# zju3dv/disprcnn

Measured on AMD Instinct MI355X. Metric: ROI cost-volumes/sec (112x112x48), higher is better.
Workload: dtype f32 (every convolution of the regressor, the three 32->1 heads included: split-f16 -- each fp32 value carried as hi + lo fp16, 3 f16-MFMA products per fp32 product, f32 accumulate; fp32-class error, tests/test_hip_s16.py.  Head gather and soft-argmin: f32 VALU); 1 GPU; Config A: per ROI pair, features [32,28,28]x2 -> concat cost volume [64,12,28,28] (folded into the first 3D layer's loads, never written) -> 3D stacked-hourglass regressor -> trilinear x4 + softmax + soft-argmin -> disparity [112,112]; maxdisp=48, mindisp=0, parallelism=roi-shard x1 (no collective), weights=closed-form synthetic (disprcnn_amd.utils.synth), BN stats calibrated fixture

## Files before the change

disprcnn_amd/csrc/convs16.hip:

```cpp
#include <hip/hip_runtime.h>
#include <stdint.h>

#include <type_traits>

#include "../../include/disprcnn_hip.h"
#include "s16_cvrows.h"
#include "s16_ovf.h"
#include "s16_tilemap.h"

typedef float f32x4 __attribute__((ext_vector_type(4)));
typedef float f32x16 __attribute__((ext_vector_type(16)));
typedef unsigned u32x4 __attribute__((ext_vector_type(4)));
typedef unsigned u32x2 __attribute__((ext_vector_type(2)));
typedef _Float16 f16x8 __attribute__((ext_vector_type(8)));
typedef _Float16 f16x4 __attribute__((ext_vector_type(4)));

#define GLOBAL_PTR(p) ((const __attribute__((address_space(1))) void*)(p))
#define LDS_PTR(p) ((__attribute__((address_space(3))) void*)(p))
#define S16_WAITCNT(vm, lgkm) (((vm) & 15) | (7 << 4) | ((lgkm) << 8) | (((vm) >> 4) << 14))

namespace {

constexpr int PV_ROWS = 128;
constexpr int PV_FLAT = 192;
constexpr int RING = 3;

template <int KW, bool CV, int RT_ = 1, int WT = 28, bool RES = false, bool Y32 = false, bool HEAD = false>
__global__ __launch_bounds__(256) __attribute__((amdgpu_waves_per_eu(1, 1))) void convs16_kernel(const drc_s16conv_params p) {
    constexpr bool FL = RT_ == 0;
    constexpr int RT = FL ? 1 : RT_;
    static_assert(!HEAD || (KW == 2 && !CV && RT == 1 && !RES && !Y32), "the fused cout-1 head is a form of the 32 -> 32 full-resolution layer");
    static_assert(!CV || (KW == 4 && RT == 1 && WT == 28 && !RES && !Y32), "the cost-volume form: 64 virtual input channels, full-resolution rows, RS16 output");
    extern __shared__ __attribute__((aligned(16))) char lds[];
    if constexpr (CV) {
        s16cv::s16_cvrows_run<1>(p, lds);
        return;
    }
    constexpr int TX = WT;
    constexpr int SX = WT + 2;
    constexpr int RPW = 4 / KW;
    constexpr int CBI = KW / 2;
    constexpr int SROWS = RPW * RT + 2;
    static_assert(RT * WT <= 32, "tile shape");
    static_assert(!FL || (KW == 2 && !CV && WT == 28 && !Y32 && !HEAD), "flat tiles: the plain / residual 32 -> 32 layer on 28-column maps");
    constexpr int PV = FL ? PV_FLAT : PV_ROWS;
    constexpr int CPB = PV * 16;
    constexpr int NH = PV / 64;
    constexpr int SLAB = CBI * 8 * CPB;
    constexpr int NL = CBI * 8 * NH / 4;
    constexpr int OWN = 16 / KW;
    constexpr int XW = 4096;
    constexpr int NR = RES ? 2 : 0;
    constexpr int NS = 2;
    static_assert(!(Y32 && (KW != 2 || RES)), "the blocked fp32 output exists for the 32-channel layers without residual");
    static_assert(FL || (RT == 1 ? SROWS * SX + 4 <= PV : (SROWS + 1) * SX + 4 <= PV), "slab plane too small (incl. the rows / columns the idle lanes over-read)");
    char* ring = lds;
    char* xchg = lds + RING * SLAB;
    char* pbuf = xchg + 2 * 4 * XW;

    const int wave = __builtin_amdgcn_readfirstlane(threadIdx.x >> 6);
    const int lane = threadIdx.x & 63;
    const int n_ = lane & 31, g = lane >> 5;
    const S16TileLane tln = s16_tile_lane<RT, WT>(n_, !(p.lo4 & 0x100));
    const int rl = tln.rl, xl = tln.xl;
    const int r = wave / KW, k = wave % KW;
    const int n_ct = p.cout / 32;
    const int ct = (int)((blockIdx.x >> 3) % n_ct);

    const int D = p.D, H = p.H, W = p.W;
    const int Wp = W + 2, Hp = H + 2;
    const long rowB = (long)Wp * 128;
    const long planeB = (long)Hp * rowB;
    const long xcbB = (long)(D + 2) * planeB;
    const long xnB = (long)CBI * xcbB;
    const int cbo = p.cout / 32;
    const long ynB = (long)cbo * xcbB;
    const long b_rowB = (long)Wp * 64, b_planeB = (long)Hp * b_rowB, b_cbB = (long)(D + 2) * b_planeB, b_nB = (long)(p.cout / 16) * b_cbB;

    f16x8 wh[27], wl[27];
    {
        const char* wb = (const char*)p.w + ((long)(ct * KW + k) * 54) * 1024 + lane * 16;
#pragma unroll
        for (int t = 0; t < 27; ++t) {
            wh[t] = *(const f16x8*)(wb + (t * 2) * 1024);
            wl[t] = *(const f16x8*)(wb + (t * 2 + 1) * 1024);
        }
    }
    constexpr int PIN_WH = 14;
#pragma unroll
    for (int t = 0; t < 27; ++t) {
        asm volatile("" : "+a"(wl[t]));
        if (t < PIN_WH) asm volatile("" : "+a"(wh[t]));
    }
    float sc[OWN], sh[OWN];
#pragma unroll
    for (int e = 0; e < OWN; ++e) {
        const int reg = k * OWN + e;
        const int co = ct * 32 + (reg & 3) + 8 * (reg >> 2) + 4 * g;
        sc[e] = p.scale[co];
        sh[e] = p.shift[co];
    }
    f16x8 w1h = {}, w1l = {};
    if constexpr (HEAD) {
        const char* wb = (const char*)p.w1 + (long)k * 2048 + lane * 16;
        w1h = *(const f16x8*)wb;
        w1l = *(const f16x8*)(wb + 1024);
    }
    int srcrow[2], srcx[2];
    bool srcok[2];
#pragma unroll
    for (int h = 0; h < 2; ++h) {
        const int v = h * 64 + lane;
        srcok[h] = v < SROWS * SX;
        const int rr = srcok[h] ? v / SX : 0;
        srcrow[h] = rr;
        srcx[h] = srcok[h] ? v - rr * SX : 0;
    }
    const unsigned bfrag0 = (unsigned)(((k >> 1) * 8 + (k & 1) * 2 + g) * CPB);
    const unsigned bfrag = bfrag0 + (unsigned)(((r * RT + rl) * SX + xl) * 16);
    const __attribute__((address_space(3))) char* ringl = (const __attribute__((address_space(3))) char*)ring;
    typedef const __attribute__((address_space(3))) f16x8 lds_frag;

    const int n_xt = (W + TX - 1) / TX, n_yt = (H + RPW * RT - 1) / (RPW * RT);
    const int Dw = (D + 2) / 3 * 3;
    const unsigned xcd = blockIdx.x & 7, qx = (blockIdx.x >> 3) / n_ct, per_xcd = (gridDim.x >> 3) / n_ct;
    const int HW = H * W, Hp1 = H + 1;
    const unsigned G = FL ? ((p.dil & 0x4000) ? 1u : 4u) : 1u;
    const unsigned cols_unit = FL ? (G * (unsigned)HW + 63u) / 64u : (unsigned)n_yt * n_xt;

    struct Col { unsigned n; int y0, x0; bool valid; int rem0, lim; };
    auto col_of = [&](unsigned it) __attribute__((always_inline)) {
        const unsigned j = it * per_xcd + qx;
        const unsigned nl = j / cols_unit;
        const unsigned rem = j - nl * cols_unit;
        if constexpr (FL) {
            Col c;
            const unsigned n0 = (nl * 8 + xcd) * G;
            const int gu = n0 < (unsigned)p.N ? (int)((unsigned)p.N - n0 < G ? (unsigned)p.N - n0 : G) : 0;
            const int f0 = (int)rem * 64;
            const int u0 = f0 / HW;
            c.valid = f0 < gu * HW;
            c.n = n0 + (unsigned)u0;
            c.rem0 = f0 - u0 * HW;
            c.lim = gu * HW - f0;
            c.y0 = c.rem0 / WT;
            c.x0 = c.rem0 - c.y0 * WT;
            return c;
        }
        const int yb = (int)(rem / n_xt), xt = (int)(rem - (unsigned)yb * n_xt);
        Col c;
        c.n = nl * 8 + xcd;
        c.valid = c.n < (unsigned)p.N;
        c.y0 = yb * RPW * RT;
        c.x0 = xt * TX;
        c.rem0 = c.lim = 0;
        return c;
    };
    struct Src { const char* a; unsigned v0, v1, v2, v3; };
    auto src_of = [&](const Col& c) __attribute__((always_inline)) {
        Src q;
        q.a = (const char*)p.x + (long)c.n * xnB;
        q.v2 = q.v3 = 0u;
        if constexpr (FL) {
            const int el = c.rem0 + (c.lim < 64 ? c.lim : 64) - 1;
            const int du_l = (el >= HW) + (el >= 2 * HW) + (el >= 3 * HW);
            const int rr_last = du_l * Hp1 + (el - du_l * HW) / WT - c.y0 + 2;
            static_assert(NH <= 4, "pieces of a chunk plane");
            unsigned vv[4] = {0u, 0u, 0u, 0u};
#pragma unroll
            for (int h = 0; h < NH; ++h) {
                const int v = h * 64 + lane;
                const int rr = v / SX, xs = v - rr * SX;
                const int L = c.y0 + rr, M = L - 1;
                const int uo = (M >= Hp1) + (M >= 2 * Hp1) + (M >= 3 * Hp1);
                const unsigned off = (unsigned)((long)uo * xnB + (long)(L - uo * Hp1) * rowB + (long)xs * 16);
                vv[h] = rr <= rr_last ? off : 0x80000000u;
            }
            q.v0 = vv[0]; q.v1 = vv[1]; q.v2 = vv[2]; q.v3 = vv[3];
            return q;
        }
        q.v0 = (unsigned)((long)(c.y0 + srcrow[0]) * rowB + (long)(c.x0 + srcx[0]) * 16);
        q.v1 = (unsigned)((long)(c.y0 + srcrow[1]) * rowB + (long)(c.x0 + srcx[1]) * 16);
        return q;
    };
    auto stage = [&](const Src& q, int pl, int slot) __attribute__((always_inline)) {
        char* dst = ring + slot * SLAB;
        const __amdgpu_buffer_rsrc_t ra = __builtin_amdgcn_make_buffer_rsrc((void*)q.a, 0, 0x7FFFFF00, 0x00020000);
        const unsigned va[4] = {q.v0, q.v1, q.v2, q.v3};
#pragma unroll
        for (int i = 0; i < NL; ++i) {
            const int id = wave * NL + i;
            const int cb = FL ? 0 : id >> 4, c = FL ? wave * (NL / NH) + i / NH : (id >> 1) & 7, h = FL ? i % NH : id & 1;
            const int so = (int)((long)cb * xcbB + (long)(pl + 1) * planeB + (long)c * (Wp * 16));
            __builtin_amdgcn_raw_ptr_buffer_load_lds(ra, LDS_PTR(dst + (cb * 8 + c) * CPB + h * 1024), 16, va[h], so, 0, 0);
        }
    };
    const bool hrows = HEAD && p.head_rows;
    const int hs_slotB = hrows ? 16 : 48;
    const long hs_planeB = (long)H * W * hs_slotB, hs_nB = (long)D * hs_planeB;
    const bool hs_drop0 = hrows && g, hs_drop1 = hrows || g;
    struct Ctx { char* y16b; char* y32b; const char* resb; char* hsb; unsigned o16, o32, ohs, bf; bool ok; };
    auto ctx_of = [&](const Col& c) __attribute__((always_inline)) {
        Ctx q;
        q.bf = bfrag;
        if constexpr (FL) {
            q.hsb = (char*)p.w;
            q.y32b = (char*)p.w;
            q.ohs = q.o32 = 0u;
            q.y16b = (char*)p.y16 + (long)c.n * ynB;
            q.resb = p.res ? (const char*)p.res + (long)c.n * ynB : (const char*)p.w;
            q.ok = r * 32 + n_ < c.lim;
            const int e0 = q.ok ? c.rem0 + r * 32 + n_ : c.rem0;
            const int du = (e0 >= HW) + (e0 >= 2 * HW) + (e0 >= 3 * HW);
            const int e = e0 - du * HW;
            const int yl = e / WT, xv = e - yl * WT;
            q.bf = bfrag0 + (unsigned)(((du * Hp1 + yl - c.y0) * SX + xv) * 16);
            q.o16 = (unsigned)((long)du * ynB + (long)ct * xcbB + planeB + (long)(yl + 1) * rowB + (long)(k * 2 + g) * (Wp * 16) + (long)(xv + 1) * 16);
            return q;
        }
        q.hsb = HEAD ? (char*)p.head + (long)c.n * hs_nB : (char*)p.w;
        q.ohs = (unsigned)(((long)(c.y0 + r * RT + rl) * W + (c.x0 + xl)) * hs_slotB + (hrows ? 0 : g * 32));
        q.y16b = p.y16 ? (char*)p.y16 + (long)c.n * ynB : (char*)p.w;
        q.y32b = p.y32 ? (char*)p.y32 + (long)c.n * b_nB : (char*)p.w;
        q.resb = p.res ? (const char*)p.res + (long)c.n * ynB : (const char*)p.w;
        const int yl = c.y0 + r * RT + rl;
        q.ok = tln.ok && yl < H && c.x0 + xl < W;
        if constexpr (KW == 2) {
            q.o16 = (unsigned)((long)ct * xcbB + planeB + (long)(yl + 1) * rowB + (long)(k * 2 + g) * (Wp * 16) + (long)(c.x0 + xl + 1) * 16);
            q.o32 = (unsigned)((long)(2 * ct + k) * b_cbB + b_planeB + (long)(yl + 1) * b_rowB + (long)(c.x0 + xl + 1) * 64 + g * 16);
        } else {
            q.o16 = (unsigned)((long)ct * xcbB + planeB + (long)(yl + 1) * rowB + (long)((k >> 1) * 2 + g) * (Wp * 16) + (long)(c.x0 + xl + 1) * 16 + (k & 1) * 8);
            q.o32 = (unsigned)((long)(2 * ct + (k >> 1)) * b_cbB + b_planeB + (long)(yl + 1) * b_rowB + (long)(c.x0 + xl + 1) * 64 + (k & 1) * 32 + g * 16);
        }
        return q;
    };
    const unsigned lo_off = (unsigned)(4 * Wp * 16);
    const float relu_lo = p.relu ? 0.f : -65504.f;
    const unsigned n16 = p.y16 ? 0x7FFFFF00u : 0u, n32 = p.y32 ? 0x7FFFFF00u : 0u, nres = p.res ? 0x7FFFFF00u : 0u;

    Col ccur = col_of(0);
    if (!ccur.valid) return;
    S16Ovf og;
#pragma unroll
    for (int e = 0; e < OWN; ++e) { og.see_raw(sc[e], 3.0e38f); og.see_raw(sh[e], 3.0e38f); }
    Src s_cur = src_of(ccur), s_next = s_cur;
    Ctx cx_cur = ctx_of(ccur), cx_prev = cx_cur;
    cx_prev.ok = false;

    f32x16 acc[3];
    u32x4 resv[3][2];
#pragma unroll
    for (int a_ = 0; a_ < 3; ++a_)
#pragma unroll
        for (int e = 0; e < 16; ++e) acc[a_][e] = 0.f;
#pragma unroll
    for (int a_ = 0; a_ < 3; ++a_) resv[a_][0] = resv[a_][1] = (u32x4){0u, 0u, 0u, 0u};
    f32x16 pkeep = {};
    float SC[5] = {0.f, 0.f, 0.f, 0.f, 0.f}, SB[5] = {0.f, 0.f, 0.f, 0.f, 0.f};
    auto head_pack = [&](const float* o) __attribute__((always_inline)) {
        const bool live = n_ < WT;
        int v_[5];
#pragma unroll
        for (int j = 0; j < 5; ++j) v_[j] = __builtin_bit_cast(int, live ? o[j] : 0.f);
        auto left = [](int a) __attribute__((always_inline)) { return __builtin_bit_cast(float, __builtin_amdgcn_update_dpp(0, a, 0x138, 0xf, 0xf, true)); };
        auto right = [](int a) __attribute__((always_inline)) { return __builtin_bit_cast(float, __builtin_amdgcn_update_dpp(0, a, 0x130, 0xf, 0xf, true)); };
        auto own = [](int a) __attribute__((always_inline)) { return __builtin_bit_cast(float, a); };
        const float a0 = (left(v_[0]) + own(v_[1])) + right(v_[2]);
        const float a1 = left(v_[3]) + own(v_[4]);
        const float b0 = right(v_[0]);
        const float b1 = (left(v_[1]) + own(v_[2])) + right(v_[3]);
        const unsigned x0 = __builtin_amdgcn_permlane32_swap(__builtin_bit_cast(unsigned, b0), 0u, false, false)[1];
        const unsigned x1 = __builtin_amdgcn_permlane32_swap(__builtin_bit_cast(unsigned, b1), 0u, false, false)[1];
        u32x4 d;
        d[0] = hrows ? __builtin_bit_cast(unsigned, a0) : __builtin_bit_cast(unsigned, o[0]);
        d[1] = hrows ? __builtin_bit_cast(unsigned, a1) : __builtin_bit_cast(unsigned, o[1]);
        d[2] = hrows ? x0 : __builtin_bit_cast(unsigned, o[2]);
        d[3] = hrows ? x1 : __builtin_bit_cast(unsigned, o[3]);
        return d;
    };
    stage(s_cur, 0, 0);
    stage(s_cur, 1 < D ? 1 : D, 1);
    __builtin_amdgcn_s_waitcnt(S16_WAITCNT(NL, 15));
    unsigned gs = 0;

    auto step = [&](int t, auto JT, auto KT) __attribute__((always_inline)) {
        constexpr int J = decltype(JT)::value;
        constexpr int KIND = decltype(KT)::value;
        constexpr bool COMPUTE = KIND != 3;
        constexpr int A0 = (J + 1) % 3, A1 = J, A2 = (J + 2) % 3;
        asm volatile("" ::: "memory");
        __builtin_amdgcn_s_waitcnt(S16_WAITCNT(NL + NS + NR, 0));
        __builtin_amdgcn_s_barrier();
        asm volatile("" ::: "memory");
        const bool fcur = t >= 2, pcur = t >= 1;
        const int qf = fcur ? t - 2 : Dw - 2 + t, qp = pcur ? t - 1 : Dw - 1;
        const __amdgpu_buffer_rsrc_t resr = __builtin_amdgcn_make_buffer_rsrc((void*)(pcur ? cx_cur.resb : cx_prev.resb), 0, nres, 0x00020000);
        const unsigned p_o16 = pcur ? cx_cur.o16 : cx_prev.o16;
        const bool p_ok = (pcur ? cx_cur.ok : cx_prev.ok) && qp >= 0 && qp < D;
        if constexpr (RES) {
            const unsigned po = p_ok ? (unsigned)((long)qp * planeB) : 0x80000000u;
            if constexpr (KW == 2) {
                resv[J][0] = __builtin_amdgcn_raw_buffer_load_b128(resr, p_o16 + po, 0, 0);
                resv[J][1] = __builtin_amdgcn_raw_buffer_load_b128(resr, p_o16 + lo_off + po, 0, 0);
            } else {
                const u32x2 a_ = __builtin_amdgcn_raw_buffer_load_b64(resr, p_o16 + po, 0, 0);
                const u32x2 b_ = __builtin_amdgcn_raw_buffer_load_b64(resr, p_o16 + lo_off + po, 0, 0);
                resv[J][0] = (u32x4){a_.x, a_.y, 0u, 0u};
                resv[J][1] = (u32x4){b_.x, b_.y, 0u, 0u};
            }
        }
        {
            const int tp = t + 2;
            const bool nxt = tp >= Dw;
            Src q;
            q.a = nxt ? s_next.a : s_cur.a;
            q.v0 = nxt ? s_next.v0 : s_cur.v0;
            q.v1 = nxt ? s_next.v1 : s_cur.v1;
            q.v2 = nxt ? s_next.v2 : s_cur.v2;
            q.v3 = nxt ? s_next.v3 : s_cur.v3;
            int pl = nxt ? tp - Dw : tp;
            pl = pl < D ? pl : D;
            stage(q, pl, (J + 2) % 3);
        }
        const __amdgpu_buffer_rsrc_t y16r = __builtin_amdgcn_make_buffer_rsrc(fcur ? cx_cur.y16b : cx_prev.y16b, 0, n16, 0x00020000);
        const __amdgpu_buffer_rsrc_t y32r = __builtin_amdgcn_make_buffer_rsrc(fcur ? cx_cur.y32b : cx_prev.y32b, 0, n32, 0x00020000);
        const unsigned f_o16 = fcur ? cx_cur.o16 : cx_prev.o16, f_o32 = fcur ? cx_cur.o32 : cx_prev.o32;
        const bool f_ok = (fcur ? cx_cur.ok : cx_prev.ok) && qf >= 0 && qf < D;
        f32x4 part[4];
        {
            const char* xb = xchg + ((gs - 1) & 1) * (4 * XW) + (r * KW) * XW + lane * 16;
            if constexpr (KW == 2) {
                part[0] = *(const f32x4*)(xb + (k * 2) * 1024);
                part[1] = *(const f32x4*)(xb + XW + (k * 2) * 1024);
                part[2] = *(const f32x4*)(xb + (k * 2 + 1) * 1024);
                part[3] = *(const f32x4*)(xb + XW + (k * 2 + 1) * 1024);
            } else {
#pragma unroll
                for (int q = 0; q < 4; ++q) part[q] = *(const f32x4*)(xb + q * XW + k * 1024);
            }
        }
        f32x4 pin[4];
        if constexpr (HEAD) {
            const char* pb = pbuf + ((gs - 1) & 1) * (2 * XW) + r * XW + lane * 16;
#pragma unroll
            for (int q = 0; q < 4; ++q) pin[q] = *(const f32x4*)(pb + q * 1024);
        }
        if constexpr (RES) {
            __builtin_amdgcn_s_waitcnt(S16_WAITCNT(2 * NL + NS + NR, 15));
            __builtin_amdgcn_sched_barrier(0);
        }
        float v[OWN];
        _Float16 vh[OWN], vl[OWN];
        const unsigned long long og_keep = S16Ovf::lanes(f_ok);
        auto fin = [&](int e) __attribute__((always_inline)) {
            float s_;
            if constexpr (KW == 2) s_ = part[(e >> 2) * 2][e & 3] + part[(e >> 2) * 2 + 1][e & 3];
            else s_ = (part[0][e] + part[1][e]) + (part[2][e] + part[3][e]);
            float x_ = s_ * sc[e] + sh[e];
            if constexpr (RES) {
                const _Float16 rh = __builtin_bit_cast(f16x8, resv[(J + 2) % 3][0])[e], rl_ = __builtin_bit_cast(f16x8, resv[(J + 2) % 3][1])[e];
                x_ += (float)rh + (float)rl_;
            }
            x_ = __builtin_amdgcn_fmed3f(x_, relu_lo, 65504.f);
            og.see(x_, og_keep);
            v[e] = x_;
            vh[e] = (_Float16)x_;
            vl[e] = (_Float16)(x_ - (float)vh[e]);
        };
        auto stores = [&]() __attribute__((always_inline)) {
            if constexpr (Y32) {
// ... 25 lines not shown
#pragma unroll
            for (int e = 0; e < 16; ++e) acc[A2][e] = 0.f;
        };
        float o_[5];
        f32x16 z_ = {};
        f16x8 bh_ = {}, bl_ = {};
        auto head_update = [&](int jj) __attribute__((always_inline)) {
            if constexpr (HEAD) {
                const bool first = t == 3;
                const float p0 = pkeep[3 * jj] + pin[(3 * jj) >> 2][(3 * jj) & 3];
                const float p1 = pkeep[3 * jj + 1] + pin[(3 * jj + 1) >> 2][(3 * jj + 1) & 3];
                const float p2 = pkeep[3 * jj + 2] + pin[(3 * jj + 2) >> 2][(3 * jj + 2) & 3];
                o_[jj] = SC[jj] + (first ? 0.f : p2);
                SC[jj] = (first ? 0.f : SB[jj]) + p1;
                SB[jj] = p0;
            }
        };
        auto head_store = [&]() __attribute__((always_inline)) {
            if constexpr (HEAD) {
                const bool scur = t >= 4;
                const int ps = scur ? t - 4 : Dw - 4 + t;
                const bool ok_ = k == 0 && (scur ? cx_cur.ok : cx_prev.ok) && ps >= 0 && ps < D;
                const __amdgpu_buffer_rsrc_t hsr = __builtin_amdgcn_make_buffer_rsrc(scur ? cx_cur.hsb : cx_prev.hsb, 0, 0x7FFFFF00, 0x00020000);
                const unsigned oh_ = scur ? cx_cur.ohs : cx_prev.ohs;
                const unsigned po = ok_ ? (unsigned)((long)ps * hs_planeB) : 0x80000000u;
                __builtin_amdgcn_raw_buffer_store_b128(head_pack(o_), hsr, oh_ + (hs_drop0 ? 0x80000000u : po), 0, 0);
                __builtin_amdgcn_raw_buffer_store_b32(__builtin_bit_cast(unsigned, o_[4]), hsr, oh_ + 16 + (hs_drop1 ? 0x80000000u : po), 0, 0);
            }
        };
        auto head_mfma = [&](int i) __attribute__((always_inline)) {
            if constexpr (HEAD) {
                if (i == 0) {
#pragma unroll
                    for (int e = 0; e < 8; ++e) { bh_[e] = vh[e]; bl_[e] = vl[e]; }
                    z_ = __builtin_amdgcn_mfma_f32_32x32x16_f16(w1h, bh_, z_, 0, 0, 0);
                } else if (i == 1) {
                    z_ = __builtin_amdgcn_mfma_f32_32x32x16_f16(w1h, bl_, z_, 0, 0, 0);
                } else {
                    z_ = __builtin_amdgcn_mfma_f32_32x32x16_f16(w1l, bh_, z_, 0, 0, 0);
                    pkeep = z_;
                    if (k == 1) {
                        char* pb = pbuf + (gs & 1) * (2 * XW) + r * XW + lane * 16;
#pragma unroll
                        for (int q = 0; q < 4; ++q) *(f32x4*)(pb + q * 1024) = (f32x4){z_[q * 4], z_[q * 4 + 1], z_[q * 4 + 2], z_[q * 4 + 3]};
                    }
                }
            }
        };
        if constexpr (COMPUTE) {
            constexpr bool K0 = KIND != 2, K2 = KIND != 1;
            const __attribute__((address_space(3))) char* sb = ringl + J * SLAB + (FL ? cx_cur.bf : bfrag);
            f16x8 bh[2], bl[2];
            bh[0] = *(lds_frag*)(sb);
            bl[0] = *(lds_frag*)(sb + 4 * CPB);
#pragma unroll
            for (int q = 0; q < 9; ++q) {
                const int kh = q / 3, kw = q - kh * 3;
                if (q + 1 < 9) {
                    const int kh1 = (q + 1) / 3, kw1 = (q + 1) - kh1 * 3;
                    bh[(q + 1) & 1] = *(lds_frag*)(sb + (kh1 * SX + kw1) * 16);
                    bl[(q + 1) & 1] = *(lds_frag*)(sb + 4 * CPB + (kh1 * SX + kw1) * 16);
                }
                const f16x8 h_ = bh[q & 1], l_ = bl[q & 1];
                const int t0 = kh * 3 + kw, t1 = 9 + t0, t2 = 18 + t0;
                if (q == OWN && !HEAD) stores();
                if (q < 8) {
                    if (K0) acc[A0] = __builtin_amdgcn_mfma_f32_32x32x16_f16(wh[t0], h_, acc[A0], 0, 0, 0);
                    acc[A1] = __builtin_amdgcn_mfma_f32_32x32x16_f16(wh[t1], h_, acc[A1], 0, 0, 0);
                    if (K2) acc[A2] = __builtin_amdgcn_mfma_f32_32x32x16_f16(wh[t2], h_, acc[A2], 0, 0, 0);
                    if (K0) acc[A0] = __builtin_amdgcn_mfma_f32_32x32x16_f16(wh[t0], l_, acc[A0], 0, 0, 0);
                    acc[A1] = __builtin_amdgcn_mfma_f32_32x32x16_f16(wh[t1], l_, acc[A1], 0, 0, 0);
                    if (K2) acc[A2] = __builtin_amdgcn_mfma_f32_32x32x16_f16(wh[t2], l_, acc[A2], 0, 0, 0);
                    if (K0) acc[A0] = __builtin_amdgcn_mfma_f32_32x32x16_f16(wl[t0], h_, acc[A0], 0, 0, 0);
                    acc[A1] = __builtin_amdgcn_mfma_f32_32x32x16_f16(wl[t1], h_, acc[A1], 0, 0, 0);
                    if (K2) acc[A2] = __builtin_amdgcn_mfma_f32_32x32x16_f16(wl[t2], h_, acc[A2], 0, 0, 0);
                    if (q < OWN) fin(q);
                    if (q < 5) head_update(q);
                    if (q == 5) head_store();
                    __builtin_amdgcn_sched_barrier(0);
                } else {
                    if (K2) acc[A2] = __builtin_amdgcn_mfma_f32_32x32x16_f16(wh[t2], h_, acc[A2], 0, 0, 0);
                    if (K0) acc[A0] = __builtin_amdgcn_mfma_f32_32x32x16_f16(wh[t0], h_, acc[A0], 0, 0, 0);
                    head_mfma(0);
                    if (K2) acc[A2] = __builtin_amdgcn_mfma_f32_32x32x16_f16(wh[t2], l_, acc[A2], 0, 0, 0);
                    acc[A1] = __builtin_amdgcn_mfma_f32_32x32x16_f16(wh[t1], h_, acc[A1], 0, 0, 0);
                    if (K2) acc[A2] = __builtin_amdgcn_mfma_f32_32x32x16_f16(wl[t2], h_, acc[A2], 0, 0, 0);
                    __builtin_amdgcn_sched_barrier(0);
                    head_mfma(1);
                    if (K0) acc[A0] = __builtin_amdgcn_mfma_f32_32x32x16_f16(wh[t0], l_, acc[A0], 0, 0, 0);
                    acc[A1] = __builtin_amdgcn_mfma_f32_32x32x16_f16(wh[t1], l_, acc[A1], 0, 0, 0);
                    if (K0) acc[A0] = __builtin_amdgcn_mfma_f32_32x32x16_f16(wl[t0], h_, acc[A0], 0, 0, 0);
                    acc[A1] = __builtin_amdgcn_mfma_f32_32x32x16_f16(wl[t1], h_, acc[A1], 0, 0, 0);
                    publish();
                    head_mfma(2);
                }
            }
        } else {
#pragma unroll
            for (int e = 0; e < OWN; ++e) fin(e);
            if constexpr (HEAD) {
#pragma unroll
                for (int jj = 0; jj < 5; ++jj) head_update(jj);
                head_store();
                head_mfma(0); head_mfma(1); head_mfma(2);
            } else {
                stores();
            }
            publish();
        }
        ++gs;
    };
    using I0 = std::integral_constant<int, 0>;
    using I1 = std::integral_constant<int, 1>;
    using I2 = std::integral_constant<int, 2>;
    using I3 = std::integral_constant<int, 3>;
#pragma unroll 1
    for (unsigned it = 0;; ++it) {
        const Col cnext = col_of(it + 1);
        s_next = cnext.valid ? src_of(cnext) : s_cur;
        step(0, I0{}, I1{});
        step(1, I1{}, I0{});
        if (Dw == 3) {
            step(2, I2{}, I2{});
        } else {
            step(2, I2{}, I0{});
#pragma unroll 1
            for (int t0 = 3; t0 + 3 < Dw; t0 += 3) {
                step(t0, I0{}, I0{});
                step(t0 + 1, I1{}, I0{});
                step(t0 + 2, I2{}, I0{});
            }
            step(Dw - 3, I0{}, I0{});
            step(Dw - 2, I1{}, I0{});
            step(Dw - 1, I2{}, I2{});
        }
        if (!cnext.valid) break;
        cx_prev = cx_cur;
        cx_cur = ctx_of(cnext);
        s_cur = s_next;
    }
    step(Dw, I0{}, I3{});
    step(Dw + 1, I1{}, I3{});
    if constexpr (HEAD) {
        step(Dw + 2, I2{}, I3{});
        const bool ok_ = k == 0 && cx_cur.ok;
        const __amdgpu_buffer_rsrc_t hsr = __builtin_amdgcn_make_buffer_rsrc(cx_cur.hsb, 0, 0x7FFFFF00, 0x00020000);
        const unsigned po = ok_ ? (unsigned)((long)(D - 1) * hs_planeB) : 0x80000000u;
        __builtin_amdgcn_raw_buffer_store_b128(head_pack(SC), hsr, cx_cur.ohs + (hs_drop0 ? 0x80000000u : po), 0, 0);
        __builtin_amdgcn_raw_buffer_store_b32(__builtin_bit_cast(unsigned, SC[4]), hsr, cx_cur.ohs + 16 + (hs_drop1 ? 0x80000000u : po), 0, 0);
    }
    og.flush(p.ovf);
}

inline long s16_flat_columns(const drc_s16conv_params& p) {
    const long G = (p.dil & 0x4000) ? 1 : 4;
    return (p.N + G - 1) / G * ((G * p.H * p.W + 63) / 64);
}
constexpr long FLAT_MIN_COLUMNS = 2048;

template <int KW, bool CV, int RT, int WT, bool RES, bool Y32, bool HEAD = false>
int launch2(const drc_s16conv_params& p, hipStream_t stream) {
    constexpr int CBI = KW / 2;
    constexpr bool FLAT = RT == 0;
    constexpr int SLAB = CBI * 8 * (FLAT ? PV_FLAT : PV_ROWS) * 16;
    constexpr int XW = 4096;
    constexpr size_t lds = CV ? (size_t)s16cv::LDS_BYTES : RING * SLAB + 2 * 4 * XW + (HEAD ? 2 * 2 * XW : 0);
    static_assert(lds <= 160 * 1024, "LDS");
    static bool attr_done = false;
    if (!attr_done) {
        (void)hipFuncSetAttribute((const void*)convs16_kernel<KW, CV, RT, WT, RES, Y32, HEAD>, hipFuncAttributeMaxDynamicSharedMemorySize, 160 * 1024);
        attr_done = true;
    }
    constexpr int rows = FLAT ? 1 : (4 / KW) * RT;
    const long columns = FLAT ? s16_flat_columns(p) : (long)p.N * ((p.H + rows - 1) / rows) * ((p.W + WT - 1) / WT);
    const int n_ct = p.cout / 32;
    long blocks = 256;
    while (blocks > 8 * n_ct && blocks / (2 * n_ct) >= columns) blocks /= 2;
    if constexpr (CV) blocks = s16cv::s16_cvrows_blocks<1>(p);
    hipLaunchKernelGGL((convs16_kernel<KW, CV, RT, WT, RES, Y32, HEAD>), dim3((unsigned)blocks), dim3(256), lds, stream, p);
    return (int)hipGetLastError();
}

template <int KW, bool CV, int RT = 1, int WT = 28>
int launch(const drc_s16conv_params& p, hipStream_t stream) {
    if (p.head) {
        if constexpr (KW == 2 && !CV && RT == 1) return launch2<KW, CV, RT, WT, false, false, true>(p, stream);
        else return -4;
    }
    if (p.y32) {
        if constexpr (KW == 2 && !CV && RT == 1) return launch2<KW, CV, RT, WT, false, true>(p, stream);
        else return -4;
    }
    if constexpr (CV) return launch2<KW, CV, RT, WT, false, false>(p, stream);
    else return p.res ? launch2<KW, CV, RT, WT, true, false>(p, stream) : launch2<KW, CV, RT, WT, false, false>(p, stream);
}

}

extern "C" int drc_conv3d_k3_s16_supported(int cin, int cout, int D, int H, int W) {
    if (cin != 32 && cin != 64) return 0;
    if (cout != 32 && cout != 64) return 0;
    return D > 0 && H > 0 && W > 0;
}

extern "C" int drc_conv3d_k3_s16_flat(const drc_s16conv_params* pp) {
    if (!pp) return -1;
    const drc_s16conv_params& p = *pp;
    const bool forced = p.dil & 0x2000;
    const long unit16 = (long)(p.D + 2) * (p.H + 2) * (p.W + 2) * 128;
    const bool can = p.cin == 32 && p.cout == 32 && p.W == 28 && p.D > 0 && p.H > 0 && p.N > 0 && p.x && p.y16 && !p.y32 && !p.head && !p.left && !p.right &&
                     4 * unit16 < 0x7FFFFF00L;
    if (p.dil & 0x1000) return forced ? -1 : 0;
    if (!can) return forced ? -4 : 0;
    if (!forced && s16_flat_columns(p) < FLAT_MIN_COLUMNS) return 0;
    return (p.dil & 0x4000) ? 1 : 4;
}

extern "C" int drc_conv3d_k3_s16_fwd(const drc_s16conv_params* pp, void* stream) {
    if (!pp) return -1;
    const drc_s16conv_params& p = *pp;
    const bool cv = p.left || p.right;
    if (!p.w || !p.scale || !p.shift) return -1;
    if (p.head) {
        if (!p.w1 || p.y16 || p.y32 || p.res || cv) return -1;
        if (p.cin != 32 || p.cout != 32 || p.W % 28 || p.D < 6 || p.D % 3) return -4;
        if (p.head_rows && p.W != 28) return -4;
        if ((long)p.D * p.H * p.W * 48 >= 0x7FFFFF00L) return -5;
    } else if (p.head_rows) return -1;
    else if (!p.y16 == !p.y32) return -1;
    if (p.y32 && (p.res || p.cin != 32 || p.W <= 14)) return -4;
    if (cv && p.res) return -4;
    if (cv ? (!p.left || !p.right || p.cin != 64) : !p.x) return -1;
    if (p.N < 0) return -2;
    if (!drc_conv3d_k3_s16_supported(p.cin, p.cout, p.D, p.H, p.W)) return -4;
    if (cv && p.W <= 14) return -4;
    if (p.N == 0) return 0;
    const long unit16 = (long)(p.cout / 32) * (p.D + 2) * (p.H + 2) * (p.W + 2) * 128;
    if (unit16 >= 0x7FFFFF00L / 2) return -5;
    hipStream_t s = (hipStream_t)stream;
    if (drc_conv3d_k3_s16_wide(pp)) return drc_conv3d_k3_s16_wide_fwd(pp, stream);
    if (cv) return launch<4, true>(p, s);
    const int flat = drc_conv3d_k3_s16_flat(pp);
    if (flat < 0) return flat;
    if (flat) return p.res ? launch2<2, false, 0, 28, true, false>(p, s) : launch2<2, false, 0, 28, false, false>(p, s);
    if (p.W <= 7) return p.cin == 32 ? launch<2, false, 4, 7>(p, s) : launch<4, false, 4, 7>(p, s);
    if (p.W <= 14) return p.cin == 32 ? launch<2, false, 2, 14>(p, s) : launch<4, false, 2, 14>(p, s);
    return p.cin == 32 ? launch<2, false>(p, s) : launch<4, false>(p, s);
}
```

disprcnn_amd/engine.py:

```python
import ctypes as C
import math

import torch

from . import _lib
from ._lib import DrcTapconvParams

CB = 16
SLACK_FLOATS = 1 << 16
LDS_PER_WAVE_MAX = 38 * 1024
MAX_SLOTS = 112
TIMING = None
SLIDE = {"enabled": True, "max_slots": 112, "ct": 2, "min_od": 3, "min_share": 1, "min_units": 700, "min_units_ct1": 150}


def _stream_ptr(device):
    return C.c_void_p(torch.cuda.current_stream(device).cuda_stream)


def _ptr(t):
    return C.c_void_p(t.data_ptr()) if t is not None else C.c_void_p(0)


def require_gpu(t, what):
# ... 1055 lines not shown


C16_TILE = {"enabled": True}


def walk2_takes(cb, OD, OH, cw):
    return cb == 2 and OD >= 4 and cw in (2, 4) and OH % (7 * (4 // cw)) == 0


def x16_rows(OH, cw, stride, cb=1):
    rg = 4 // cw
    if stride == 0:
        big, small = 7, 2
        if cb * 2 * (7 * rg + 1) * 1024 + 1024 > 80 * 1024:
            return small
    elif stride == 1:
        big, small = 7, 2
    else:
        big, small = {1: 7, 2: 4, 4: 2}[rg], (1 if rg == 4 else 2)
    pad = lambda rw: -(-OH // (rw * rg)) * rw * rg
    return big if pad(big) * 4 <= pad(small) * 5 else small


class ConvPlan16:

    def __init__(self, x, y_geom, classes, in_mul, out_mul, grid_dhw, cout, relu, dense1=False):
        p = DrcTapconvParams()
        OD, OH, OW = grid_dhw
        p.N, p.OD, p.OH, p.OW = x.N, OD, OH, OW
        p.in_mul, p.out_mul = in_mul, out_mul
        p.cb_in = x.cb
        p.cout_pad = (cout + CB - 1) // CB * CB
        p.relu = int(relu)
        p.n_classes = len(classes)
        p.R, p.WT = choose_tile16(OH, OW)
        p.reserved = 1 if dense1 else 0
        for ci, c in enumerate(classes):
            k = p.cls[ci]
            k.nd, k.nh, k.nw = c["n"]
            k.dd0, k.dh0, k.dw0 = c["first"]
            k.sd, k.sh, k.sw = c["step"]
            k.wbase = c["wbase"]
            k.wsd, k.wsh, k.wsw = c["wstep"]
            k.out_off_d, k.out_off_h, k.out_off_w = c["off"]
        self.p, self.device, self.dense1 = p, x.device, dense1
        ntaps = sum(c["n"][0] * c["n"][1] * c["n"][2] for c in classes)
        self.flops = 2 * x.N * OD * OH * OW * ntaps * x.C * cout
        self.kname = "conv16_kernel<%d,%d>" % (min(-(-(p.R * p.WT) // 16), 4), 2 if (p.cout_pad // 16) % 2 == 0 else 1)
        self.tile = bool(C16_TILE["enabled"] and _lib.lib().drc_conv16_k3_tile_supported(C.byref(p)))
        ct = p.cout_pad // 16
        cw = 4 if ct % 4 == 0 else (2 if ct % 2 == 0 else 1)
        if self.tile:
            rw = 4 if (OH % 16 == 0 or OH >= 48) else 2
            if classes[0]["n"][0] == 3 and x.cb == 1 and p.cout_pad <= 32 and OD >= 4:
                self.kname = "conv16s_kernel<%d,%d>" % (rw, ct)
                if OH % 28 == 0 or OH % 16 == 0:
                    self.kname = "conv16sp_kernel<%d,%d>" % (7 if OH % 28 == 0 else 4, ct)
            elif classes[0]["n"][0] == 3 and not dense1:
                self.kname = "conv16d_kernel<%d,%d,1>" % (x16_rows(OH, cw, 1), cw)
                if walk2_takes(x.cb, OD, OH, cw):
                    self.kname = "conv16sw_kernel<7,%d>" % cw
            else:
                self.kname = "conv16t_kernel<%d,%d,%d>" % (rw, cw, classes[0]["n"][0])
        self.costvol_lo4 = None
        self.tile_x = None
        if C16_TILE["enabled"] and not self.tile and not dense1:
            if _lib.lib().drc_conv16_k3s2_tile_supported(C.byref(p)):
                self.tile_x = "drc_conv16_k3s2_tile_fwd"
                self.kname = "conv16d_kernel<%d,%d,2>" % (x16_rows(OH, cw, 2), cw)
            elif _lib.lib().drc_deconv16_k3s2_tile_supported(C.byref(p)):
                self.tile_x = "drc_deconv16_k3s2_tile_fwd"
                self.kname = "conv16u_kernel<%d,%d,%d>" % (x16_rows(OH, cw, 0, x.cb), cw, x.cb)

    def run(self, x, w16, scale, shift, y, res=None):
        p = self.p
        p.x, p.w = x.storage.data_ptr(), w16.data_ptr()
        p.x_n_stride, p.x_cb_stride, p.x_d_stride, p.x_h_stride = x.n_stride, x.cb_stride, x.d_stride, x.h_stride
        if self.dense1:
            p.y = y.data_ptr()
            p.res = res.data_ptr() if res is not None else None
            p.scale = p.shift = None
        else:
            p.y = y.storage.data_ptr()
            p.y_n_stride, p.y_cb_stride, p.y_d_stride, p.y_h_stride = y.n_stride, y.cb_stride, y.d_stride, y.h_stride
            p.y_off0 = y.interior_off
            p.scale, p.shift = scale.data_ptr(), shift.data_ptr()
            if res is not None:
                p.res = res.storage.data_ptr()
                p.r_n_stride, p.r_cb_stride, p.r_d_stride, p.r_h_stride = res.n_stride, res.cb_stride, res.d_stride, res.h_stride
                p.r_off0 = res.interior_off
            else:
                p.res = None
        if TIMING is not None:
            e0, e1 = torch.cuda.Event(enable_timing=True), torch.cuda.Event(enable_timing=True)
            e0.record(torch.cuda.current_stream(self.device))
        if self.costvol_lo4 is not None:
            st = _lib.lib().drc_conv16_k3_costvol_fwd(C.byref(p), self.costvol_lo4, _stream_ptr(self.device))
            _lib.check(st, "drc_conv16_k3_costvol_fwd")
        elif self.tile:
            st = _lib.lib().drc_conv16_k3_tile_fwd(C.byref(p), _stream_ptr(self.device))
            _lib.check(st, "drc_conv16_k3_tile_fwd")
        elif self.tile_x:
            st = getattr(_lib.lib(), self.tile_x)(C.byref(p), _stream_ptr(self.device))
            _lib.check(st, self.tile_x)
        else:
            st = _lib.lib().drc_conv16_fwd(C.byref(p), _stream_ptr(self.device))
            _lib.check(st, "drc_conv16_fwd")
        if TIMING is not None:
            e1.record(torch.cuda.current_stream(self.device))
            TIMING.append((self.kname, self.flops, e0, e1))


def plan_conv3d16(x, y, stride, cout, relu):
    assert (x.pd, x.ph, x.pw) == (1, 1, 1)
    return ConvPlan16(x, y, taps_conv((3, 3, 3), (1, 1, 1), (1, 1, 1), (1, 1, 1)), stride, 1, (y.D, y.H, y.W), cout, relu)


COSTVOL16_FUSED = {"enabled": True}


def plan_conv3d16_costvol(pair, y, lo4, cout, relu):
    assert (pair.pd, pair.ph, pair.pw) == (1, 1, 1) and pair.C == 64 and pair.D == 1 and (pair.H, pair.W) == (y.H, y.W)
    pl = ConvPlan16(pair, y, taps_conv((3, 3, 3), (1, 1, 1), (1, 1, 1), (1, 1, 1)), 1, 1, (y.D, y.H, y.W), cout, relu)
    pl.costvol_lo4, pl.tile, pl.tile_x = int(lo4), False, None
    ct = pl.p.cout_pad // 16
    cw = 4 if ct % 4 == 0 else (2 if ct % 2 == 0 else 1)
    pl.kname = "conv16d_kernel<%d,%d,1,cv>" % (x16_rows(y.H, cw, 1), cw)
    if walk2_takes(2, y.D, y.H, cw):
        pl.kname = "conv16sw_kernel<7,%d,cv>" % cw
    pl.flops = 2 * y.N * y.D * y.H * y.W * 27 * 64 * cout
    return pl


def plan_deconv3d16(x, y, cout, relu):
    assert (x.pd, x.ph, x.pw) == (1, 1, 1) and (y.D, y.H, y.W) == (2 * x.D, 2 * x.H, 2 * x.W)
    return ConvPlan16(x, y, taps_deconv3d_k3s2(), 1, 2, (x.D, x.H, x.W), cout, relu)


def plan_conv3d16_cout1(x):
    return ConvPlan16(x, None, taps_conv((3, 3, 3), (1, 1, 1), (1, 1, 1), (1, 1, 1)), 1, 1, (x.D, x.H, x.W), 1, False, dense1=True)


def cost_volume16_blocked(left, right, out, lo4, hi4, in_blocked_pad=-1):
    st = _lib.lib().drc_cost_volume16_blocked_fwd(_ptr(left), _ptr(right), _ptr(out.storage), out.N, out.C // 2, out.D, out.H, out.W,
                                                  lo4, hi4, in_blocked_pad, _stream_ptr(out.device))
    _lib.check(st, "drc_cost_volume16_blocked_fwd")


HEAD_FUSED = {"enabled": True}
LASTCONV_S16 = {"enabled": True}
S16 = {"enabled": True}
HEAD_ROWS = {"enabled": True}
FLAT_TILES = {"enabled": True, "group": 4}
CV_WIDE = {"enabled": True}



_GUARD = {"cur": None, "safe": False}


class OverflowPolicy:

    def __init__(self, cap=256):
        self.cap, self.level, self.skip, self.overflows, self.checks = cap, 0, 0, 0, 0

    def want_fast(self):
        if self.skip > 0:
            self.skip -= 1
            return False
        return True

    def report(self, overflowed):
        self.checks += 1
        if overflowed:
            self.overflows += 1
            self.skip = min(1 << self.level, self.cap)
            self.level = min(self.level + 1, 30)
        else:
            self.level = 0


class OverflowGuard:

    def __init__(self, device):
        self.word = torch.zeros(1, dtype=torch.int32, device=device)
        self.policy = OverflowPolicy()
        self.used = False
        self.warned = False
        self.dirty = False

    def ptr(self):
        self.used = True
        return C.c_void_p(self.word.data_ptr())

    def tripped(self):
        v = int(self.word.item())
        if v:
            self.word.zero_()
        return bool(v)


_SHARED_GUARDS = {}


def one_guard(fn, device, what="guarded call", enabled=True):
    dev = torch.device(device)
    g = _SHARED_GUARDS.get(dev)
    if g is None:
        g = _SHARED_GUARDS[dev] = OverflowGuard(dev)
    return guarded(g, fn, what=what, enabled=enabled)


def s16_allowed():
    return not _GUARD["safe"]


def _ovf_ptr():
    g = _GUARD["cur"]
    return g.ptr() if g is not None else None


def guard_in_scope():
    return _GUARD["cur"]


def guarded(guard, fn, strict=False, what="split-f16 path", enabled=True):
    if _GUARD["cur"] is not None or guard is None or not enabled or (torch.cuda.is_available() and torch.cuda.is_current_stream_capturing()):
        return fn()
    import warnings
    pol = guard.policy
    if getattr(guard, "dirty", False):
        guard.word.zero_()
        guard.dirty = False
    _GUARD["cur"], _GUARD["safe"] = guard, (False if strict else not pol.want_fast())
    guard.used = False
    try:
        try:
            out = fn()
        except BaseException:
            if guard.used:
                guard.dirty = True
            raise
        if not guard.used:
            return out
        over = guard.tripped()
        pol.report(over)
        if not over:
            return out
        if strict:
            raise RuntimeError(f"{what}: a value left the split-f16 range (|v| > 65504, Inf or NaN) and math = 'f16x2' was requested; use "
                               f"'auto' (re-runs on the fp32 kernels) or 'f32'")
        if not guard.warned:
            guard.warned = True
            warnings.warn(f"{what}: a value left the split-f16 range (|v| > 65504, Inf or NaN); this pass and the next {pol.skip} run on the "
                          f"fp32 kernels (reference arithmetic, config/defaults.py:22).  Reported once per model.", RuntimeWarning, stacklevel=3)
        _GUARD["safe"] = True
        guard.used = False
        out = fn()
        if guard.used and guard.tripped():
            raise RuntimeError(f"{what}: the fp32 re-run still issued split-f16 launches that overflowed")
        return out
    finally:
        _GUARD["cur"], _GUARD["safe"] = None, False


class RS16:

    def __init__(self, N, C_, D, H, W, pd, device, storage=None):
        if C_ % 32:
            raise ValueError("RS16: channels must be a multiple of 32")
        self.N, self.C, self.D, self.H, self.W, self.pd = N, C_, D, H, W, pd
        self.cb = C_ // 32
        self.unit = self.cb * (D + 2 * pd) * (H + 2) * 8 * (W + 2) * 8
        self.numel = N * self.unit
        slack = self.slack = max(4096, 8 * 8 * (W + 2) * 8)
        if storage is None:
            self.storage = torch.zeros(self.numel + slack, dtype=torch.float16, device=device)
        else:
            if storage.numel() < self.numel + slack:
                raise ValueError("RS16: the given storage is too small for this geometry")
            self.storage = storage.narrow(0, 0, self.numel + slack)
        self.device = device

    def view7(self):
        return self.storage[: self.numel].view(self.N, self.cb, self.D + 2 * self.pd, self.H + 2, 8, self.W + 2, 8)

    def from_dense(self, dense):
        require_gpu(dense, "RS16.from_dense")
        dense = dense.contiguous()
        if self.N:
            st = _lib.lib().drc_rs16_from_dense(_ptr(dense), _ptr(self.storage), self.N, self.C, self.D, self.H, self.W, self.pd, _ovf_ptr(), _stream_ptr(self.device))
            _lib.check(st, "drc_rs16_from_dense")
        return self

    def from_blocked(self, blk, first_unit=0):
        base = getattr(blk, "base", blk)
        if (blk.C, blk.D, blk.H, blk.W) != (self.C, self.D, self.H, self.W) or base.N < first_unit + self.N:
            raise ValueError("RS16.from_blocked: shapes differ")
        if self.N:
            src = C.c_void_p(base.storage.data_ptr() + 4 * first_unit * base.n_stride)
            st = _lib.lib().drc_rs16_from_blocked(src, _ptr(self.storage), self.N, self.C, self.D, self.H, self.W, base.pd, base.ph, base.pw, base.cb,
                                                  getattr(blk, "cb_off", 0), self.pd, _ovf_ptr(), _stream_ptr(self.device))
            _lib.check(st, "drc_rs16_from_blocked")
        return self

    def to_blocked(self, blk, first_unit=0):
        base = getattr(blk, "base", blk)
        if (blk.C, blk.D, blk.H, blk.W) != (self.C, self.D, self.H, self.W) or base.N < first_unit + self.N:
            raise ValueError("RS16.to_blocked: shapes differ")
        if self.N:
            dst = C.c_void_p(base.storage.data_ptr() + 4 * first_unit * base.n_stride)
            st = _lib.lib().drc_rs16_to_blocked(_ptr(self.storage), dst, self.N, self.C, self.D, self.H, self.W, base.pd, base.ph, base.pw, base.cb,
                                                getattr(blk, "cb_off", 0), self.pd, _stream_ptr(self.device))
            _lib.check(st, "drc_rs16_to_blocked")
        return blk

    def to_dense(self):
        shape = (self.N, self.C, self.D, self.H, self.W)
        out = torch.empty(shape, dtype=torch.float32, device=self.device)
        if self.N:
            st = _lib.lib().drc_rs16_to_dense(_ptr(self.storage), _ptr(out), self.N, self.C, self.D, self.H, self.W, self.pd, _stream_ptr(self.device))
            _lib.check(st, "drc_rs16_to_dense")
        return out


def s16_supported(cin, cout, D, H, W, kind="s1", dil=1):
    if kind == "2d":
        return bool(S16["enabled"] and D == 1 and _lib.lib().drc_conv2d_k3_s16_supported(cin, cout, H, W, dil))
    fn = {"s1": "drc_conv3d_k3_s16_supported", "s2": "drc_conv3d_k3s2_s16_supported", "up": "drc_deconv3d_k3s2_s16_supported"}[kind]
    return bool(S16["enabled"] and getattr(_lib.lib(), fn)(cin, cout, D, H, W))


class ConvPlanS16:

    def __init__(self, N, cin, cout, D, H, W, relu, cv=False, device=None, kind="s1", dil=1):
        if not s16_supported(cin, cout, D, H, W, kind, dil) or (cv and (cin != 64 or kind != "s1" or W <= 14)) or (dil != 1 and kind != "2d"):
            raise ValueError("ConvPlanS16: unsupported shape")
        self.dil = dil
        self.N, self.cin, self.cout, self.D, self.H, self.W, self.relu, self.cv, self.device, self.kind = N, cin, cout, D, H, W, bool(relu), cv, device, kind
        self.out_dhw = {"s1": (D, H, W), "s2": (D // 2, H // 2, W // 2), "up": (2 * D, 2 * H, 2 * W), "2d": (1, H, W)}[kind]
        self.pd = 0 if kind == "2d" else 1
        vox = D * H * W if kind != "s2" else (D // 2) * (H // 2) * (W // 2)
        self.flops = 2 * N * vox * (9 if kind == "2d" else 27) * cin * cout
        rt, wt = (1, 28)
        nw = {"s1": W, "s2": W // 2, "up": W, "2d": W}[kind]
        if nw <= 14:
            rt, wt = (2, 14) if nw > 7 else (4, 7)
        if kind == "s1":
            self._kfmt = "convs16_kernel<%d,%s,%d,%d,%%s,%%s,%%s>" % (cin // 16, "true" if cv else "false", rt, wt)
            self.kname = self._kfmt % ("false", "false", "false")
            from ._lib import DrcS16ConvParams
            probe = DrcS16ConvParams(None if cv else 1, 1, 1, 1, None, 1, None, 1 if cv else None, 1 if cv else None, N, D, H, W, cin, cout, int(bool(relu)), 0, 1)
            self._wide_ok = bool(_lib.lib().drc_conv3d_k3_s16_wide(C.byref(probe)))
            self._wname = "convs16w_kernel<%d,%s>" % (cin // 16, "true" if cv else "false")
            if self._wide:
                self.kname = self._wname
        elif kind == "2d":
            wide = cin == 64 and W % 56 == 0 and cout == 128 and N * (H // 28) * (W // 56) * (cout // 32) >= 256
            kw, ks = {32: (2, 1), 128: (4, 2)}.get(cin, (2, 2) if wide else (4, 1))
            self._kfmt = "convs16r_kernel<%d,%d,%%s,%d>" % (kw, ks, dil)
            self.kname = self._kfmt % "false"
        elif kind == "s2":
            cs = cin == 32 and cout == 64
            ring = 3 if (cs or (cin == 32 and nw == 14)) else 2
            self.kname = "convs16d_kernel<%d,%d,%d,%d,true,%s>" % (cin // 16, rt, wt, ring, "true" if cs else "false")
        else:
            self.kname = "convs16u_kernel<%d,%d>" % (rt, wt)

    @property
    def _wide(self):
        return self.kind == "s1" and self._wide_ok and bool(CV_WIDE["enabled"])

    def _flat_bits(self):
        if self.kind != "s1" or self.cv:
            return 0
        if not FLAT_TILES["enabled"]:
            return 0x1000
        return (0x2000 if FLAT_TILES.get("force") else 0) | (0x4000 if int(FLAT_TILES["group"]) == 1 else 0)

    def run(self, x16, w16, scale, shift, y16=None, y32=None, res=None, left=None, right=None, lo4=0, head=None, head_rows=False):
        from ._lib import DrcS16ConvParams
        if head is not None:
            if self.kind != "s1" or self.cv or (self.cin, self.cout) != (32, 32) or self.W % 28 or self.D < 6 or self.D % 3 or y16 is not None or y32 is not None or res is not None:
                raise ValueError("ConvPlanS16.run: the fused head is the 32 -> 32 full-resolution layer without another output")
            if head[1].dtype != torch.float32 or head[1].numel() < self.N * self.D * self.H * self.W * (4 if head_rows else 12) or head[0].dtype != torch.float16 or head[0].numel() != 2048:
                raise ValueError("ConvPlanS16.run: head = (halfs [2][2][64][8], fp32 buffer of N*D*H*W*12; rows layout: *4)")
        elif head_rows:
            raise ValueError("ConvPlanS16.run: head_rows is a layout of the fused head")
        if x16 is not None and (x16.N < self.N or (x16.C, x16.D, x16.H, x16.W, x16.pd) != (self.cin, self.D, self.H, self.W, self.pd)):
            raise ValueError("ConvPlanS16.run: input geometry differs from the plan")
        for t_ in (y16, res):
            if t_ is not None and (t_.N < self.N or (t_.C, t_.D, t_.H, t_.W, t_.pd) != (self.cout,) + self.out_dhw + (self.pd,)):
                raise ValueError("ConvPlanS16.run: output / residual geometry differs from the plan")
        if self.kind == "2d" and (y16 is None or y32 is not None or x16 is None):
            raise ValueError("ConvPlanS16.run: the 2D kernel reads and writes RS16 maps")
        if y32 is not None and (self.kind != "s1" or (y32.C, y32.D, y32.H, y32.W, y32.pd, y32.ph, y32.pw) != (self.cout, self.D, self.H, self.W, 1, 1, 1) or getattr(y32, "cb_off", 0)):
            raise ValueError("ConvPlanS16.run: the blocked fp32 output (stride-1 kernel only) must be a whole tensor with halo 1")
        if self.kind != "s1" and (y16 is None or (res is not None and self.kind == "s2")):
            raise ValueError("ConvPlanS16.run: the stride-2 / transposed kernels write RS16 (the stride-2 one takes no residual)")
        if self.cv:
            for f in (left, right):
                if f is None or (f.C, f.D, f.H, f.W, f.pd) != (32, 1, self.H, self.W, 0) or f.N < self.N:
                    raise ValueError("ConvPlanS16.run: the cost-volume variant reads two RS16 2D maps [N,32,H,W]")
        elif x16 is None:
            raise ValueError("ConvPlanS16.run: input missing")
        p = DrcS16ConvParams(_ptr(x16.storage) if x16 is not None else None, _ptr(w16), _ptr(scale), _ptr(shift),
                             _ptr(res.storage) if res is not None else None, _ptr(y16.storage) if y16 is not None else None,
                             _ptr(y32.storage) if y32 is not None else None, _ptr(left.storage) if self.cv else None,
                             _ptr(right.storage) if self.cv else None, self.N, self.D, self.H, self.W, self.cin, self.cout, int(self.relu), int(lo4),
                             0x800 if (self.cv and self.kind == "s1" and not CV_WIDE["enabled"]) else int(self.dil) | self._flat_bits(),
                             _ptr(head[1]) if head is not None else None, _ptr(head[0]) if head is not None else None, _ovf_ptr(), int(bool(head_rows)))
        dev = self.device
        if TIMING is not None:
            e0, e1 = torch.cuda.Event(enable_timing=True), torch.cuda.Event(enable_timing=True)
            e0.record(torch.cuda.current_stream(dev))
        fn = {"s1": "drc_conv3d_k3_s16_fwd", "s2": "drc_conv3d_k3s2_s16_fwd", "up": "drc_deconv3d_k3s2_s16_fwd", "2d": "drc_conv2d_k3_s16_fwd"}[self.kind]
        st = getattr(_lib.lib(), fn)(C.byref(p), _stream_ptr(dev))
        _lib.check(st, fn)
        if TIMING is not None:
            e1.record(torch.cuda.current_stream(dev))
            if self.kind == "s1" and self._wide and res is None and y32 is None and head is None:
                kn = self._wname
            elif self.kind == "s1":
                kn = self._kfmt % ("true" if res is not None else "false", "true" if y32 is not None else "false", "true" if head is not None else "false")
            elif self.kind == "2d":
                kn = self._kfmt % ("true" if res is not None else "false")
            else:
                kn = self.kname
            TIMING.append((kn, self.flops + (2 * 27 * 32 * self.N * self.D * self.H * self.W if head is not None else 0), e0, e1))
```

Measured before the change: 63990 ROI cost-volumes/s.

## Extend flat-tile path to 64->64 convolutions on 14-column maps

Result: faster. 64760 ROI cost-volumes/s (median of 6 runs) (+1.2%).

```diff
diff --git a/disprcnn_amd/csrc/convs16.hip b/disprcnn_amd/csrc/convs16.hip
--- a/disprcnn_amd/csrc/convs16.hip
+++ b/disprcnn_amd/csrc/convs16.hip
@@ -42,8 +42,9 @@
     constexpr int CBI = KW / 2;
     constexpr int SROWS = RPW * RT + 2;
     static_assert(RT * WT <= 32, "tile shape");
-    static_assert(!FL || (KW == 2 && !CV && WT == 28 && !Y32 && !HEAD), "flat tiles: the plain / residual 32 -> 32 layer on 28-column maps");
-    constexpr int PV = FL ? PV_FLAT : PV_ROWS;
+    static_assert(!FL || (((KW == 2 && WT == 28) || (KW == 4 && WT == 14)) && !CV && !Y32 && !HEAD), "flat tiles: the plain / residual 32 -> 32 layer on 28-column maps, 64 -> 64 on 14-column maps");
+    constexpr int FV = 32 * RPW;
+    constexpr int PV = FL && KW == 2 ? PV_FLAT : PV_ROWS;
     constexpr int CPB = PV * 16;
     constexpr int NH = PV / 64;
     constexpr int SLAB = CBI * 8 * CPB;
@@ -125,8 +126,8 @@
     const int Dw = (D + 2) / 3 * 3;
     const unsigned xcd = blockIdx.x & 7, qx = (blockIdx.x >> 3) / n_ct, per_xcd = (gridDim.x >> 3) / n_ct;
     const int HW = H * W, Hp1 = H + 1;
-    const unsigned G = FL ? ((p.dil & 0x4000) ? 1u : 4u) : 1u;
-    const unsigned cols_unit = FL ? (G * (unsigned)HW + 63u) / 64u : (unsigned)n_yt * n_xt;
+    const unsigned G = FL ? ((p.dil & 0x4000) ? 1u : (KW == 4 && (p.dil & 0x8000)) ? 8u : 4u) : 1u;
+    const unsigned cols_unit = FL ? (G * (unsigned)HW + (unsigned)(FV - 1)) / (unsigned)FV : (unsigned)n_yt * n_xt;
 
     struct Col { unsigned n; int y0, x0; bool valid; int rem0, lim; };
     auto col_of = [&](unsigned it) __attribute__((always_inline)) {
@@ -137,7 +138,7 @@
             Col c;
             const unsigned n0 = (nl * 8 + xcd) * G;
             const int gu = n0 < (unsigned)p.N ? (int)((unsigned)p.N - n0 < G ? (unsigned)p.N - n0 : G) : 0;
-            const int f0 = (int)rem * 64;
+            const int f0 = (int)rem * FV;
             const int u0 = f0 / HW;
             c.valid = f0 < gu * HW;
             c.n = n0 + (unsigned)u0;
@@ -162,7 +163,7 @@
         q.a = (const char*)p.x + (long)c.n * xnB;
         q.v2 = q.v3 = 0u;
         if constexpr (FL) {
-            const int el = c.rem0 + (c.lim < 64 ? c.lim : 64) - 1;
+            const int el = c.rem0 + (c.lim < FV ? c.lim : FV) - 1;
             const int du_l = (el >= HW) + (el >= 2 * HW) + (el >= 3 * HW);
             const int rr_last = du_l * Hp1 + (el - du_l * HW) / WT - c.y0 + 2;
             static_assert(NH <= 4, "pieces of a chunk plane");
@@ -190,7 +191,8 @@
 #pragma unroll
         for (int i = 0; i < NL; ++i) {
             const int id = wave * NL + i;
-            const int cb = FL ? 0 : id >> 4, c = FL ? wave * (NL / NH) + i / NH : (id >> 1) & 7, h = FL ? i % NH : id & 1;
+            const int fc = wave * (NL / NH) + i / NH;
+            const int cb = FL ? (CBI == 1 ? 0 : fc >> 3) : id >> 4, c = FL ? (CBI == 1 ? fc : fc & 7) : (id >> 1) & 7, h = FL ? i % NH : id & 1;
             const int so = (int)((long)cb * xcbB + (long)(pl + 1) * planeB + (long)c * (Wp * 16));
             __builtin_amdgcn_raw_ptr_buffer_load_lds(ra, LDS_PTR(dst + (cb * 8 + c) * CPB + h * 1024), 16, va[h], so, 0, 0);
         }
@@ -215,7 +217,8 @@
             const int e = e0 - du * HW;
             const int yl = e / WT, xv = e - yl * WT;
             q.bf = bfrag0 + (unsigned)(((du * Hp1 + yl - c.y0) * SX + xv) * 16);
-            q.o16 = (unsigned)((long)du * ynB + (long)ct * xcbB + planeB + (long)(yl + 1) * rowB + (long)(k * 2 + g) * (Wp * 16) + (long)(xv + 1) * 16);
+            const int och = KW == 2 ? k * 2 + g : (k >> 1) * 2 + g, ohalf = KW == 2 ? 0 : (k & 1) * 8;
+            q.o16 = (unsigned)((long)du * ynB + (long)ct * xcbB + planeB + (long)(yl + 1) * rowB + (long)och * (Wp * 16) + (long)(xv + 1) * 16 + ohalf);
             return q;
         }
         q.hsb = HEAD ? (char*)p.head + (long)c.n * hs_nB : (char*)p.w;
@@ -547,17 +550,41 @@
     og.flush(p.ovf);
 }
 
+constexpr long FLAT_MIN_COLUMNS = 2048;
+constexpr long FLAT_HALF_GROUP = 8;
+constexpr long FLAT_HALF_MIN_COLUMNS = 1176;
+
+inline long s16_flat_group(const drc_s16conv_params& p) {
+    if (p.dil & 0x4000) return 1;
+    if (p.cin != 64) return 4;
+    return (p.dil & 0x8000) ? 8 : (p.dil & 0x10000) ? 4 : FLAT_HALF_GROUP;
+}
 inline long s16_flat_columns(const drc_s16conv_params& p) {
-    const long G = (p.dil & 0x4000) ? 1 : 4;
-    return (p.N + G - 1) / G * ((G * p.H * p.W + 63) / 64);
-}
-constexpr long FLAT_MIN_COLUMNS = 2048;
+    const long G = s16_flat_group(p), FV = p.cin == 64 ? 32 : 64;
+    return (p.N + G - 1) / G * ((G * p.H * p.W + FV - 1) / FV);
+}
+inline bool s16_flat_half_fits(long N, long G, long H) {
+    const long HW = H * 14, Hp1 = H + 1;
+    const long tail = N % G;
+    for (int pass = 0; pass < 2; ++pass) {
+        const long gu = pass == 0 ? (N >= G ? G : 0) : tail;
+        for (long f0 = 0; f0 < gu * HW; f0 += 32) {
+            const long u0 = f0 / HW, rem0 = f0 - u0 * HW, y0 = rem0 / 14;
+            const long lim = gu * HW - f0;
+            const long el = rem0 + (lim < 32 ? lim : 32) - 1;
+            const long du_l = el / HW;
+            const long rr_last = du_l * Hp1 + (el - du_l * HW) / 14 - y0 + 2;
+            if (du_l > 3 || rr_last > 7) return false;
+        }
+    }
+    return true;
+}
 
 template <int KW, bool CV, int RT, int WT, bool RES, bool Y32, bool HEAD = false>
 int launch2(const drc_s16conv_params& p, hipStream_t stream) {
     constexpr int CBI = KW / 2;
     constexpr bool FLAT = RT == 0;
-    constexpr int SLAB = CBI * 8 * (FLAT ? PV_FLAT : PV_ROWS) * 16;
+    constexpr int SLAB = CBI * 8 * (FLAT && KW == 2 ? PV_FLAT : PV_ROWS) * 16;
     constexpr int XW = 4096;
     constexpr size_t lds = CV ? (size_t)s16cv::LDS_BYTES : RING * SLAB + 2 * 4 * XW + (HEAD ? 2 * 2 * XW : 0);
     static_assert(lds <= 160 * 1024, "LDS");
@@ -603,12 +630,14 @@
     const drc_s16conv_params& p = *pp;
     const bool forced = p.dil & 0x2000;
     const long unit16 = (long)(p.D + 2) * (p.H + 2) * (p.W + 2) * 128;
-    const bool can = p.cin == 32 && p.cout == 32 && p.W == 28 && p.D > 0 && p.H > 0 && p.N > 0 && p.x && p.y16 && !p.y32 && !p.head && !p.left && !p.right &&
-                     4 * unit16 < 0x7FFFFF00L;
+    const bool half = p.cin == 64 && p.cout == 64 && p.W == 14;
+    const bool shape = (p.cin == 32 && p.cout == 32 && p.W == 28) || half;
+    const bool can = shape && p.D > 0 && p.H > 0 && p.N > 0 && p.x && p.y16 && !p.y32 && !p.head && !p.left && !p.right &&
+                     4 * (p.cout / 32) * unit16 < 0x7FFFFF00L && (!half || s16_flat_half_fits(p.N, s16_flat_group(p), p.H));
     if (p.dil & 0x1000) return forced ? -1 : 0;
     if (!can) return forced ? -4 : 0;
-    if (!forced && s16_flat_columns(p) < FLAT_MIN_COLUMNS) return 0;
-    return (p.dil & 0x4000) ? 1 : 4;
+    if (!forced && s16_flat_columns(p) < (half ? FLAT_HALF_MIN_COLUMNS : FLAT_MIN_COLUMNS)) return 0;
+    return (int)s16_flat_group(p);
 }
 
 extern "C" int drc_conv3d_k3_s16_fwd(const drc_s16conv_params* pp, void* stream) {
@@ -637,7 +666,12 @@
     if (cv) return launch<4, true>(p, s);
     const int flat = drc_conv3d_k3_s16_flat(pp);
     if (flat < 0) return flat;
-    if (flat) return p.res ? launch2<2, false, 0, 28, true, false>(p, s) : launch2<2, false, 0, 28, false, false>(p, s);
+    if (flat) {
+        drc_s16conv_params q = p;
+        q.dil = (p.dil & ~0x1C000) | (flat == 1 ? 0x4000 : flat == 8 ? 0x8000 : 0x10000);
+        if (p.cin == 64) return p.res ? launch2<4, false, 0, 14, true, false>(q, s) : launch2<4, false, 0, 14, false, false>(q, s);
+        return p.res ? launch2<2, false, 0, 28, true, false>(q, s) : launch2<2, false, 0, 28, false, false>(q, s);
+    }
     if (p.W <= 7) return p.cin == 32 ? launch<2, false, 4, 7>(p, s) : launch<4, false, 4, 7>(p, s);
     if (p.W <= 14) return p.cin == 32 ? launch<2, false, 2, 14>(p, s) : launch<4, false, 2, 14>(p, s);
     return p.cin == 32 ? launch<2, false>(p, s) : launch<4, false>(p, s);
diff --git a/disprcnn_amd/engine.py b/disprcnn_amd/engine.py
--- a/disprcnn_amd/engine.py
+++ b/disprcnn_amd/engine.py
@@ -1231,6 +1231,7 @@
 S16 = {"enabled": True}
 HEAD_ROWS = {"enabled": True}
 FLAT_TILES = {"enabled": True, "group": 4}
+FLAT_TILES_HALF = {"enabled": True, "group": 8}
 CV_WIDE = {"enabled": True}
 
 
@@ -1453,6 +1454,10 @@
     def _flat_bits(self):
         if self.kind != "s1" or self.cv:
             return 0
+        if (self.cin, self.cout, self.W) == (64, 64, 14):
+            if not FLAT_TILES_HALF["enabled"]:
+                return 0x1000
+            return (0x2000 if FLAT_TILES_HALF.get("force") else 0) | {1: 0x4000, 8: 0x8000, 4: 0x10000}[int(FLAT_TILES_HALF["group"])]
         if not FLAT_TILES["enabled"]:
             return 0x1000
         return (0x2000 if FLAT_TILES.get("force") else 0) | (0x4000 if int(FLAT_TILES["group"]) == 1 else 0)
```
